# hebench/reference-seal-backend

Measured on AMD Instinct MI355X. Metric: ciphertext-ops/sec (CKKS ct x ct mul+relin+rescale, N=2^15, L=16), higher is better.
Workload: dtype u64 (exact residues; fp64-FMA engine for primes < 2^47, u64 Harvey engine with the fold reduction for the 60-bit primes)

## Files before the change

reference-seal-backend_amd/csrc/he355_kernels.hip:

```cpp
#include <hip/hip_runtime.h>

#include <cstdio>
#include <cstdlib>
#include <stdexcept>
#include <type_traits>

#include "he355_kernels.h"
#include "ntt_core.h"
#include "client/ckks_codec.h"
#include "client/multiword.h"
#include "client/sampler.h"

#if !defined(HE355_KNS) || !defined(HE355_U64_FOLD)
#error "he355_kernels.hip is compiled once per form of the u64 engine: -DHE355_KNS=ks_shoup -DHE355_U64_FOLD=0 and -DHE355_KNS=ks_fold -DHE355_U64_FOLD=1 (Makefile)"
#endif
namespace he355 {
namespace HE355_KNS {
namespace {

#include "kernel_common.inc"

template <class Ar>
__device__ __forceinline__ void rows_fwd_job(const PrimeDev &P, u64 *row, bool in_raw, u32 rowbase, int lane, u64 *lds, bool valid)
{
// ... 309 lines not shown
{
    s0 = s1 = s2 = make_ulonglong2(0, 0);
    for (int k = 0; k < inner; ++k, pa += a_step, pb += b_step) {
        const ulonglong2 a0 = reinterpret_cast<const ulonglong2 *>(pa)[e2], a1 = reinterpret_cast<const ulonglong2 *>(pa + P1)[e2];
        const ulonglong2 b0 = reinterpret_cast<const ulonglong2 *>(pb)[e2], b1 = reinterpret_cast<const ulonglong2 *>(pb + P1)[e2];
        ulonglong2 c0, c1, c2;
        mul3_pair(ar, a0, a1, b0, b1, c0, c1, c2);
        s0.x = addmod(s0.x, c0.x, q); s0.y = addmod(s0.y, c0.y, q);
        s1.x = addmod(s1.x, c1.x, q); s1.y = addmod(s1.y, c1.y, q);
        s2.x = addmod(s2.x, c2.x, q); s2.y = addmod(s2.y, c2.y, q);
    }
}

__global__ void __launch_bounds__(kBlock) k_mul3_acc(const u64 *a, const u64 *b, u64 *out, const PrimeDev *primes, int L, int logN, u64 rows, u64 cols,
                                                     int inner, u64 a_stride_i, u64 a_stride_k, u64 b_stride_k, u64 b_stride_j)
{
    const u64 pairs_per_poly = (u64)1 << (logN - 1);
    const u64 gid = (u64)blockIdx.x * kBlock + threadIdx.x;
    const u64 ri = gid >> (logN - 1);
    const u64 e2 = gid & (pairs_per_poly - 1);
    const u64 r = ri / L;
    if (r >= rows * cols) return;
    const int i = (int)(ri % L);
    const u64 poly = (u64)1 << logN, P1 = (u64)L << logN, ct = 2 * P1;
    const u64 *pa = a + (r / cols) * a_stride_i * ct + i * poly, *pb = b + (r % cols) * b_stride_j * ct + i * poly;
    ulonglong2 s0, s1, s2;
    const PrimeDev &P = primes[i];
    if (P.f64) mul3_acc_pair(make_ar(P, (ArF64 *)nullptr), P.q, pa, pb, a_stride_k * ct, b_stride_k * ct, P1, e2, inner, s0, s1, s2);
    else mul3_acc_pair(make_ar(P, (ArU64 *)nullptr), P.q, pa, pb, a_stride_k * ct, b_stride_k * ct, P1, e2, inner, s0, s1, s2);
    u64 *po = out + r * 3 * P1 + i * poly;
    reinterpret_cast<ulonglong2 *>(po)[e2] = s0;
    reinterpret_cast<ulonglong2 *>(po + P1)[e2] = s1;
    reinterpret_cast<ulonglong2 *>(po + 2 * P1)[e2] = s2;
}

template <class Ar, int BLOCK>
__device__ __forceinline__ typename std::conditional<std::is_same<Ar, ArF64>::value, TwRowF64, TwRow>::type
stage_row_twiddles(const PrimeDev &P, const Ar &ar, u32 rowbase, unsigned char *twl_raw, bool inverse = false)
{
    constexpr bool kF64 = std::is_same<Ar, ArF64>::value;
    typename std::conditional<kF64, TwRowF64, TwRow>::type twr;
    const gtw_t gf = gtw(inverse ? P.inv : P.fwd);
    constexpr int kIter = (kRowTw + BLOCK - 1) / BLOCK;
    Tw16 tmp[kIter];
#pragma unroll
    for (int k = 0; k < kIter; ++k) {
        const u32 i = threadIdx.x + k * BLOCK;
        tmp[k] = tw_load(gf, tw_row_source(rowbase, i + 1 < (u32)kRowTw ? i : 0));
    }
    if constexpr (kF64) {
        double *twl = reinterpret_cast<double *>(twl_raw);
#pragma unroll
        for (int k = 0; k < kIter; ++k)
            if (threadIdx.x + k * BLOCK < (u32)kRowTw) twl[threadIdx.x + k * BLOCK] = ArF64::tw_w(tmp[k]);
        twr.t = twl;
        twr.qinv = ar.qinv;
    } else {
        Tw16 *twl = reinterpret_cast<Tw16 *>(twl_raw);
#pragma unroll
        for (int k = 0; k < kIter; ++k)
            if (threadIdx.x + k * BLOCK < (u32)kRowTw) twl[threadIdx.x + k * BLOCK] = tmp[k];
        twr.t = twl;
    }
    return twr;
}

constexpr int K1_MUL_C2 = 3;
struct K1Args {
    const u64 *addend;
    const u64 *a, *b;
    Indexer ix;
    const uint32_t *perm;
    u64 *c01; u64 c01_item_stride;
    u64 *c2n, *c2r;
    u64 n_ops, op_offset;
    int L, logn1, mode;
    int no_c1;
    int no_c0n;
    int n_i;
    unsigned char i_list[64];
    KsGroups groups;
};

template <class Ar, int MODE, class ITW = int>
__device__ __forceinline__ void k1_job(const K1Args &A, const PrimeDev &P, u64 op, int i, u32 a_row, int lane, u64 *lds, bool valid, const ITW *staged = nullptr)
{
    typedef typename Ar::T T;
    const Ar ar = make_ar(P, (Ar *)nullptr);
    const u32 n1 = 1u << A.logn1;
    const u64 N = (u64)n1 << kRowLog, P1 = (u64)A.L * N;
    const u64 roff = (u64)i * N + ((u64)a_row << kRowLog);
    u64 *c0p = A.c01 + op * A.c01_item_stride + roff;
    u64 *c1p = c0p + P1;
    u64 *c2np = A.c2n + op * P1 + roff;
    u64 *c2rp = A.c2r + op * P1 + roff;
    T x[kRowE];
    u64 v0[kRowE], v1[kRowE];
    if (MODE == K1_MUL || MODE == K1_MUL_C2) {
        const u64 r = A.op_offset + op;
        const u64 *pa = A.a + idx_a(A.ix, r) * 2 * P1 + roff, *pb = A.b + idx_b(A.ix, r) * 2 * P1 + roff;
        u64 a0[kRowE], a1[kRowE], b0[kRowE], b1[kRowE];
        u64 v2[kRowE];
        if (MODE == K1_MUL_C2) {
            load_rowC(pa + P1, lane, a1);
            load_rowC(pb + P1, lane, b1);
#pragma unroll
            for (int r2 = 0; r2 < kRowE; ++r2) x[r2] = ar.dy_mul(ar.dy_in(a1[r2]), ar.dy_in(b1[r2]));
        } else {
        load_rowC(pa, lane, a0); load_rowC(pa + P1, lane, a1);
        load_rowC(pb, lane, b0); load_rowC(pb + P1, lane, b1);
#pragma unroll
        for (int r2 = 0; r2 < kRowE; ++r2) {
            const T x0 = ar.dy_in(a0[r2]), x1 = ar.dy_in(a1[r2]), y0 = ar.dy_in(b0[r2]), y1 = ar.dy_in(b1[r2]);
            v0[r2] = ar.dy_out(ar.dy_mul(x0, y0));
            v1[r2] = ar.dy_out(ar.dy_add(ar.dy_mul(x0, y1), ar.dy_mul(x1, y0)));
            v2[r2] = ar.dy_out(ar.dy_mul(x1, y1));
            x[r2] = ar.from_canon(v2[r2]);
        }
        if (valid) { store_rowC(c0p, lane, v0); store_rowC(c1p, lane, v1); store_rowC(c2np, lane, v2); }
        }
    } else if (MODE == K1_CT3) {
        const u64 *pa = A.a + (A.op_offset + op) * 3 * P1 + roff;
        u64 v2[kRowE];
        load_rowC(pa + 2 * P1, lane, v2);
#pragma unroll
        for (int r2 = 0; r2 < kRowE; ++r2) x[r2] = ar.from_canon(v2[r2]);
        if (!A.no_c1) {
            load_rowC(pa, lane, v0); load_rowC(pa + P1, lane, v1);
            if (valid) { store_rowC(c0p, lane, v0); store_rowC(c1p, lane, v1); store_rowC(c2np, lane, v2); }
        }
    } else {
        u64 src_ct = A.op_offset + op;
        const uint32_t *perm = A.perm;
        if (A.groups.group_size) {
            const u32 gop = (u32)(A.op_offset + op), grp = gop / A.groups.group_size;
            src_ct = (u64)A.groups.src_block[grp] * A.groups.group_size + gop % A.groups.group_size;
            perm = A.groups.perm[grp];
        }
        const u64 *p0 = A.a + src_ct * 2 * P1 + (u64)i * N;
        const uint32_t *pm = perm + ((u64)a_row << kRowLog);
        u64 v2[kRowE];
        {
            const u64 *srow = p0 + (u64)(__builtin_amdgcn_readfirstlane(pm[0]) & ~(u32)(kRowN - 1));
            u32 pl[kRowE];
#pragma unroll
            for (int r2 = 0; r2 < kRowE; ++r2) pl[r2] = lds_pad((int)(pm[elemC(lane, r2)] & (u32)(kRowN - 1)));
            u64 t[kRowE];
            load_rowC(srow + P1, lane, t);
            lds_store_C(lds, lane, t);
            HE_WAVE_SYNC();
#pragma unroll
            for (int r2 = 0; r2 < kRowE; ++r2) v2[r2] = lds[pl[r2]];
            if (!A.no_c0n) {
                load_rowC(srow, lane, t);
                HE_WAVE_SYNC();
                lds_store_C(lds, lane, t);
                HE_WAVE_SYNC();
#pragma unroll
                for (int r2 = 0; r2 < kRowE; ++r2) v0[r2] = lds[pl[r2]];
            }
            HE_WAVE_SYNC();
#pragma unroll
            for (int r2 = 0; r2 < kRowE; ++r2) {
                if (A.no_c0n) v0[r2] = 0;
                v1[r2] = 0;
                x[r2] = ar.from_canon(v2[r2]);
            }
        }
        if (A.addend && !A.no_c0n) {
            const u64 *ad = A.addend + (A.op_offset + op) * 2 * P1 + roff;
            u64 a0[kRowE];
            load_rowC(ad, lane, a0);
            if (!A.no_c1) load_rowC(ad + P1, lane, v1);
#pragma unroll
            for (int r2 = 0; r2 < kRowE; ++r2) v0[r2] = addmod(v0[r2], a0[r2], P.q);
        }
        if (valid) {
            if (!A.no_c0n) store_rowC(c0p, lane, v0);
            if (!A.no_c1) store_rowC(c1p, lane, v1);
            store_rowC(c2np, lane, v2);
        }
    }
    const bool last = A.logn1 == 0;
    if constexpr (std::is_same<ITW, int>::value) wave_rows_inv(ar, P, last, n1 + a_row, lane, lds, x);
    else wave_rows_inv_tw(ar, *staged, P.inv_w0_scaled, last, lane, lds, x);
#pragma unroll
    for (int r2 = 0; r2 < kRowE; ++r2) v0[r2] = last ? ar.to_canon(x[r2]) : ar.to_raw(x[r2]);
    if (valid) store_rowA(c2rp, lane, v0);
}

template <int MODE, class Ar>
__global__ void __launch_bounds__(kBlock) k_k1(K1Args A, const PrimeDev *primes)
{
    __shared__ u64 lds[kWaves][kLdsRow];
    constexpr bool kF64 = std::is_same<Ar, ArF64>::value;
    __shared__ __attribute__((aligned(16))) unsigned char twl_raw[kF64 ? kRowTw * 8 : kRowTw * 16];
    const int wave = threadIdx.x >> 6, lane = threadIdx.x & 63;
    const u32 n1 = 1u << A.logn1;
    const u64 n_opg = (A.n_ops + kWaves - 1) / kWaves;
    const u64 tile = blockIdx.x / n_opg, opg = blockIdx.x % n_opg;
    const u32 a_row = (u32)(tile & (n1 - 1));
    const int i = A.i_list[tile >> A.logn1];
    u64 op = opg * kWaves + wave;
    const bool valid = op < A.n_ops;
    if (!valid) op = A.n_ops - 1;
    const PrimeDev &P = primes[i];
    const Ar ar = make_ar(P, (Ar *)nullptr);
    const auto itw = stage_row_twiddles<Ar, kBlock>(P, ar, n1 + a_row, twl_raw, true);
    __syncthreads();
    k1_job<Ar, MODE>(A, P, op, i, a_row, lane, lds[wave], valid, &itw);
}
template <int MODE, class Ar>
__device__ __forceinline__ void k1_block(const K1Args &A, const PrimeDev *primes, const unsigned bid_x, u64 (*lds)[kLdsRow])
{
    const int wave = threadIdx.x >> 6, lane = threadIdx.x & 63;
    const u32 n1 = 1u << A.logn1;
    const u64 total = A.n_ops * A.n_i * n1;
    u64 job = (u64)bid_x * kWaves + wave;
    const bool valid = job < total;
    if (!valid) job = total - 1;
    const u32 a_row = (u32)(job & (n1 - 1));
    const u64 oi = job >> A.logn1;
    const int i = A.i_list[oi % A.n_i];
    const u64 op = oi / A.n_i;
    k1_job<Ar, MODE>(A, primes[i], op, i, a_row, lane, lds[wave], valid);
}
template <int MODE>
__global__ void __launch_bounds__(kBlock) k_k1_dual(K1Args AF, K1Args AU, unsigned n_f, const PrimeDev *primes)
{
    __shared__ u64 lds[kWaves][kLdsRow];
    if (blockIdx.x < n_f) k1_block<MODE, ArF64>(AF, primes, blockIdx.x, lds);
    else k1_block<MODE, ArU64>(AU, primes, blockIdx.x - n_f, lds);
}

struct K2Args {
    const u64 *c2r;
    u64 src_op_stride;
    u64 *d;
    u64 n_ops;
    int L, K, ckks, src_is_coeff;
    u64 f64_mask;
    int n_dig;
    unsigned char dig_list[64];
    int tsplit;
};

__device__ __forceinline__ double lift_wide(const ArF64 &ar, u64 v, double pow32)
{
    return ar.mulmod_vv((double)(u32)(v >> 32), pow32) + (double)(u32)v;
}
typedef const __attribute__((address_space(4))) double *cdw_t;
__device__ __forceinline__ cdw_t cdw(const double *p) { return (cdw_t)(unsigned long long)p; }
typedef u32 u32x2_t __attribute__((ext_vector_type(2)));
constexpr u32 kSlotBytes = kRowN * 8;
__device__ __forceinline__ __amdgpu_buffer_rsrc_t poly_rsrc(const void *p, u32 bytes)
{
    const unsigned long long v = (unsigned long long)p;
    const u32 lo = __builtin_amdgcn_readfirstlane((u32)v), hi = __builtin_amdgcn_readfirstlane((u32)(v >> 32));
    return __builtin_amdgcn_make_buffer_rsrc((void *)(((unsigned long long)hi << 32) | lo), 0, (int)bytes, 0x00020000);
}
template <int N1> __device__ __forceinline__ void store_pattern_rows(__amdgpu_buffer_rsrc_t dst, u32 off4, u32 off2h, const double x[N1])
{
#pragma unroll
    for (int a = 0; a < N1; ++a) {
        union { u64 u; double d; } c;
        c.d = x[a];
        __builtin_amdgcn_raw_buffer_store_b32((u32)c.u, dst, (int)off4, a * (int)kSlotBytes, 0);
        __builtin_amdgcn_raw_buffer_store_b16((unsigned short)(c.u >> 32), dst, (int)off2h, a * (int)kSlotBytes, 0);
    }
}
template <int N1> __device__ __forceinline__ void store_word_rows(__amdgpu_buffer_rsrc_t dst, u32 off8, const u64 x[N1])
{
#pragma unroll
    for (int a = 0; a < N1; ++a) {
        u32x2_t v;
        v.x = (u32)x[a]; v.y = (u32)(x[a] >> 32);
        __builtin_amdgcn_raw_buffer_store_b64(v, dst, (int)off8, a * (int)kSlotBytes, 0);
    }
}
typedef u32 u32x4_t __attribute__((ext_vector_type(4)));
template <int N1>
__device__ __forceinline__ void store_pattern_rows_wide(__amdgpu_buffer_rsrc_t dst, unsigned char *tile, int lane, u32 lane_lo, u32 lane_hi, const double x[N1])
{
    static_assert(N1 % 8 == 0, "written for whole groups of 8 rows");
    u32 *lo = reinterpret_cast<u32 *>(tile);
    unsigned short *hi = reinterpret_cast<unsigned short *>(tile + N1 * 256);
#pragma unroll
    for (int a = 0; a < N1; ++a) {
        union { u64 u; double d; } c;
        c.d = x[a];
        lo[a * 64 + lane] = (u32)c.u;
        hi[a * 64 + lane] = (unsigned short)(c.u >> 32);
    }
// ... 1802 lines not shown
```

reference-seal-backend_amd/csrc/k3_body.inc:

```
    static_assert(!GROUPED || !TENSOR, "grouped keys are for rotations");
    constexpr int kWaves = WAVES, kBlock = WAVES * 64;
    typedef typename Ar::T T;
    typedef typename Ar::Acc Acc;
    constexpr bool kF64 = std::is_same<Ar, ArF64>::value;
    constexpr bool kPacked = kF64;
    constexpr int kDigitPieces = kPacked ? 6 : 8;
    K3_LDS_DECL
    const int wave = threadIdx.x >> 6, lane = threadIdx.x & 63;
    const u32 n1 = 1u << A.logn1;
    const u64 N = (u64)n1 << kRowLog;
    const u64 n_og = (A.n_ops + kWaves - 1) / kWaves;
    const u64 n_ogb = (n_og + A.og_per_block - 1) / A.og_per_block;
    const u64 total_tiles = (u64)A.n_tt * n1;
    const u64 s = K3_BID_X >> 3, xcd = K3_BID_X & 7;
    const u64 tile = (s / n_ogb) * 8 + xcd;
    if (tile >= total_tiles) return;
    const u64 og_first = A.og_stride > 1 ? s % n_ogb : (s % n_ogb) * A.og_per_block;
    const int tt = A.tt_list[tile >> A.logn1];
    const int q_slot = A.q_slot[tile >> A.logn1];
    const u32 a_row = (u32)(tile & (n1 - 1));
    const int t = (tt == A.L) ? A.K - 1 : tt;
    const PrimeDev &P = primes[t];
    const Ar ar = make_ar(P, (Ar *)nullptr);
    const u64 rowoff = (u64)a_row << kRowLog;
    const auto twr = stage_row_twiddles<Ar, kBlock>(P, ar, n1 + a_row, twl_raw);
    __syncthreads();
    for (u32 g = 0; g < A.og_per_block; ++g) {
        const u64 og = og_first + (u64)g * A.og_stride;
        if (og >= n_og) break;
        u64 op = og * kWaves + wave;
        const bool valid = op < A.n_ops;
        if (!valid) op = A.n_ops - 1;
        Acc acc0[kRowE], acc1[kRowE];
#pragma unroll
        for (int r = 0; r < kRowE; ++r) { acc0[r] = 0; acc1[r] = 0; }
        auto tensor_init = [&]() {
            if constexpr (TENSOR) {
                const u64 tr = A.t_op_offset + op;
                const u64 LNt = (u64)A.L * N;
                const u64 *pa = A.ta + idx_a(A.tix, tr) * 2 * LNt + (u64)tt * N + rowoff;
                const u64 *pb = A.tb + idx_b(A.tix, tr) * 2 * LNt + (u64)tt * N + rowoff;
                u64 a0[kRowE], a1[kRowE], b0[kRowE], b1[kRowE];
                load_rowC(pa, lane, a0); load_rowC(pb, lane, b0);
                load_rowC(pa + LNt, lane, a1); load_rowC(pb + LNt, lane, b1);
#pragma unroll
                for (int r = 0; r < kRowE; ++r) {
                    const T x0 = ar.dy_in(a0[r]), x1 = ar.dy_in(a1[r]), y0 = ar.dy_in(b0[r]), y1 = ar.dy_in(b1[r]);
                    acc0[r] = ar.acc_from_lazy(ar.dy_mul(x0, y0));
                    acc1[r] = ar.acc_from_lazy(ar.dy_add(ar.dy_mul(x0, y1), ar.dy_mul(x1, y0)));
                }
            }
        };
        constexpr int kRun = Ar::kAccRun;
        int pend = 0;
        auto acc_flush = [&]() {
            if constexpr (kRun > 1) {
                if (pend) {
#pragma unroll
                    for (int r = 0; r < kRowE; ++r) { acc0[r] = ar.acc_reduce(acc0[r]); acc1[r] = ar.acc_reduce(acc1[r]); }
                    pend = 0;
                }
            }
        };
        auto acc_step = [&]() {
            if constexpr (kRun > 1) {
                if (++pend == kRun) acc_flush();
            }
        };
        auto mac_row = [&](Acc acc[kRowE], const T x[kRowE], const u64 kv[kRowE], const u64 kq[kRowE]) {
#pragma unroll
            for (int r = 0; r < kRowE; ++r) {
                if constexpr (kRun > 1) ar.acc_mac_lazy(acc[r], x[r], ar.key_in(kv[r]), Ar::kKeyQuotient ? kq[r] : 0);
                else ar.acc_mac(acc[r], x[r], ar.key_in(kv[r]), Ar::kKeyQuotient ? kq[r] : 0);
            }
        };
        const u64 *kbase = A.key, *kqbase = A.keyq;
        if constexpr (GROUPED) {
            typedef const __attribute__((address_space(4))) unsigned long long *ckeys_t;
            const u32 grp = __builtin_amdgcn_readfirstlane((u32)((A.g_op_offset + op) / A.groups.group_size));
            kbase = (const u64 *)((ckeys_t)(unsigned long long)A.groups.key)[grp];
            kqbase = kbase + A.keyq_offset;
        }
        auto key_row = [&](int j, int k) -> const u64 * { return kbase + (((u64)j * 2 + k) * A.K + t) * N + rowoff; };
        auto keyq_row = [&](int j, int k) -> const u64 * { return kqbase + (((u64)j * 2 + k) * A.n_q + q_slot) * N + rowoff; };
        auto mac_poly = [&](Acc acc[kRowE], const T x[kRowE], int j, int k) {
            u64 kv[kRowE], kq[kRowE];
            load_rowC(key_row(j, k), lane, kv);
            if constexpr (Ar::kKeyQuotient) load_rowC(keyq_row(j, k), lane, kq);
            mac_row(acc, x, kv, kq);
        };
        auto mac_digit = [&](const T x[kRowE], int j) {
            mac_poly(acc0, x, j, 0);
            mac_poly(acc1, x, j, 1);
            acc_step();
        };
        auto gather_base = [&](int poly, const uint32_t *&pm) -> const u64 * {
            u64 src_ct = A.gsrc_op_offset + op;
            pm = A.gperm;
            if constexpr (GROUPED) {
                const u32 gop = (u32)(A.g_op_offset + op), gi = __builtin_amdgcn_readfirstlane(gop / A.groups.group_size);
                src_ct = (u64)A.groups.src_block[gi] * A.groups.group_size + gop % A.groups.group_size;
                pm = A.groups.perm[gi];
            }
            pm += rowoff;
            return A.gsrc + (src_ct * 2 + (u64)poly) * ((u64)A.L * N) + (u64)tt * N;
        };
        auto gather_row = [&](int poly, u64 v[kRowE]) {
            const uint32_t *pm;
            const u64 *p0 = gather_base(poly, pm);
#pragma unroll
            for (int r = 0; r < kRowE; ++r) v[r] = p0[pm[elemC(lane, r)]];
        };
        const bool has_own = A.ckks && tt < A.L;
        const int nd = A.L - (has_own ? 1 : 0);
        auto digit = [&](int i) -> int { return (has_own && i >= tt) ? i + 1 : i; };
        const int split = FUSE ? 1 : (A.n_split > 1 ? A.n_split : 1), grp = split > 1 ? (int)K3_BID_Y : 0;
        const int i_begin = nd * grp / split, i_end = nd * (grp + 1) / split;
        auto src_row = [&](int j) -> const u64 * { return A.d + ((op * (A.L + 1) + tt) * A.L + j) * N + rowoff; };
        if (i_begin < i_end) dma_row_to_lds<kDigitPieces>(src_row(digit(i_begin)), stage[wave], lane);
        tensor_init();
        if (has_own && grp == 0) {
            if constexpr (TENSOR) {
                const u64 tr = A.t_op_offset + op;
                const u64 LNt = (u64)A.L * N;
                u64 a1[kRowE], b1[kRowE];
                load_rowC(A.ta + (idx_a(A.tix, tr) * 2 + 1) * LNt + (u64)tt * N + rowoff, lane, a1);
                load_rowC(A.tb + (idx_b(A.tix, tr) * 2 + 1) * LNt + (u64)tt * N + rowoff, lane, b1);
                T x[kRowE];
#pragma unroll
                for (int r = 0; r < kRowE; ++r) x[r] = ar.dy_mul(ar.dy_in(a1[r]), ar.dy_in(b1[r]));
                mac_digit(x, tt);
            } else {
                T x[kRowE];
                u64 v[kRowE];
                load_rowC(FUSE && A.c1_mode == 3 ? A.c1_src + (op * 3 + 2) * ((u64)A.L * N) + (u64)tt * N + rowoff : A.c2n + (op * A.L + tt) * N + rowoff, lane, v);
#pragma unroll
                for (int r = 0; r < kRowE; ++r) x[r] = ar.from_canon(v[r]);
                mac_digit(x, tt);
            }
        }
        if constexpr (FUSE || TENSOR) {
            const bool resc = A.cols2 != nullptr;
            const int n_rows = nd + 2;
            const u64 LN = (u64)A.L * N, L1N = (u64)(A.L - 1) * N;
            auto row_ptr = [&](int i) -> const u64 * {
                if (i < nd) return src_row(digit(i));
                if (!resc) return A.cols + ((op * 2 + (i - nd)) * A.L + tt) * N + rowoff;
                return A.cols2 + ((op * 2 + (i - nd)) * (A.L - 1) + tt) * N + rowoff;
            };
            const FloorConst fc = A.fc[(A.K - 1) * A.K + t];
            const FloorConst fc2 = A.fc[(resc ? A.L - 1 : 0) * A.K + t];
            if (FUSE && nd == 0) dma_row_to_lds(row_ptr(0), stage[wave], lane);
            for (int i = 0; i < nd; ++i) {
                T x[1][kRowE];
                asm volatile("s_waitcnt vmcnt(0)" ::: "memory");
                if constexpr (kPacked) {
                    lds_rowA48(stage[wave], lane, x[0]);
                } else {
                    u64 v[kRowE];
                    lds_rowA(stage[wave], lane, v);
#pragma unroll
                    for (int r = 0; r < kRowE; ++r) x[0][r] = ar.from_raw(v[r]);
                }
                asm volatile("s_waitcnt lgkmcnt(0)" ::: "memory");
                if (i + 1 < nd) dma_row_to_lds<kDigitPieces>(row_ptr(i + 1), stage[wave], lane);
                else if constexpr (FUSE) dma_row_to_lds(row_ptr(i + 1), stage[wave], lane);
                if constexpr (!Ar::kKeyQuotient) {
                    u64 kv0[kRowE], kv1[kRowE];
                    const int j = digit(i);
                    wave_rows_fwd_n(ar, twr, lane, lds[wave], x, [&]() { load_rowC(key_row(j, 0), lane, kv0); load_rowC(key_row(j, 1), lane, kv1); });
                    if constexpr (kF64) {
#pragma unroll
                        for (int r0 = 0; r0 < kRowE; r0 += kMacG / 2) {
                            double xs[kMacG], ks[kMacG], pr[kMacG];
#pragma unroll
                            for (int k = 0; k < kMacG / 2; ++k) {
                                xs[2 * k] = x[0][r0 + k]; ks[2 * k] = ar.key_in(kv0[r0 + k]);
                                xs[2 * k + 1] = x[0][r0 + k]; ks[2 * k + 1] = ar.key_in(kv1[r0 + k]);
                            }
                            ar.template mulmod_vv_g<kMacG>(xs, ks, pr);
#pragma unroll
                            for (int k = 0; k < kMacG / 2; ++k) { acc0[r0 + k] += pr[2 * k]; acc1[r0 + k] += pr[2 * k + 1]; }
                        }
                    }
                } else {
                    wave_rows_fwd_n<Ar, decltype(twr), NoHook, true>(ar, twr, lane, lds[wave], x);
                    mac_digit(x[0], digit(i));
                }
            }
            acc_flush();
            constexpr bool kAccForms = TENSOR || GROUPED;
            const bool direct = kAccForms && Ar::kAccDirect && floor_direct(P.acc_terms, (u32)A.L + 2);
#pragma unroll 1
            for (int i = nd; FUSE && i < n_rows; ++i) {
                T x[1][kRowE];
                u64 v[kRowE], av[kRowE];
                asm volatile("s_waitcnt vmcnt(0)" ::: "memory");
                lds_rowA(stage[wave], lane, v);
#pragma unroll
                for (int r = 0; r < kRowE; ++r) x[0][r] = ar.from_raw(v[r]);
                asm volatile("s_waitcnt lgkmcnt(0)" ::: "memory");
                if (i + 1 < n_rows) dma_row_to_lds(row_ptr(i + 1), stage[wave], lane);
                const int k = i - nd;
                u64 *c01_row = A.c01 + op * A.c01_item_stride + k * LN + (u64)tt * N + rowoff;
                if constexpr (TENSOR) {
                } else if (k == 0 && A.c1_mode == 4) {
                    gather_row(0, av);
                } else if (k == 0 && A.c1_mode == 5) {
                    u64 ad[kRowE];
                    load_rowC(A.c1_src + (op * 2 + 0) * LN + (u64)tt * N + rowoff, lane, ad);
                    gather_row(0, av);
#pragma unroll
                    for (int r = 0; r < kRowE; ++r) av[r] = addmod(av[r], ad[r], P.q);
                } else if (k == 1 && (A.c1_mode == 1 || A.c1_mode == 4)) {
#pragma unroll
                    for (int r = 0; r < kRowE; ++r) av[r] = 0;
                } else if (A.c1_mode == 3) {
                    load_rowC(A.c1_src + (op * 3 + k) * LN + (u64)tt * N + rowoff, lane, av);
                } else {
                    load_rowC(k == 1 && (A.c1_mode == 2 || A.c1_mode == 5) ? A.c1_src + (op * 2 + 1) * LN + (u64)tt * N + rowoff : c01_row, lane, av);
                }
                bool into_sum = false;
                u64 *sum_row = nullptr;
                u32 sum_cnt = 0;
                if constexpr (GROUPED && !TENSOR) {
                    if (A.groups.sum_out) {
                        const u32 gop = (u32)(A.g_op_offset + op), gi = __builtin_amdgcn_readfirstlane(gop / A.groups.group_size);
                        sum_cnt = A.groups.count[gi];
                        sum_row = A.groups.sum_out + ((u64)(gop % A.groups.group_size) * 2 + k) * LN + (u64)tt * N + rowoff;
                        into_sum = sum_cnt == 1 && !resc;
                        if (into_sum) {
                            u64 o[kRowE];
                            load_rowC(sum_row, lane, o);
#pragma unroll
                            for (int r = 0; r < kRowE; ++r) av[r] = addmod(av[r], o[r], P.q);
                        }
                    }
                }
                if constexpr (!kF64 && Ar::kFold) {
                    wave_rows_fwd_n<Ar, decltype(twr), NoHook, true>(ar, twr, lane, lds[wave], x);
#pragma unroll
                    for (int r = 0; r < kRowE; ++r) x[0][r] = ar.lazy_reduce(x[0][r]);
                } else {
                    wave_rows_fwd_n(ar, twr, lane, lds[wave], x);
                }
                const Acc *acc = k == 0 ? acc0 : acc1;
                if (kAccForms && Ar::kAccDirect && !direct) {
                    if (k == 0) {
#pragma unroll
                        for (int r = 0; r < kRowE; ++r) ar.floor_prep(acc0[r], x[0][r]);
                    } else {
#pragma unroll
                        for (int r = 0; r < kRowE; ++r) ar.floor_prep(acc1[r], x[0][r]);
                    }
                }
                if constexpr (TENSOR) {
                    if (!resc) {
#pragma unroll
                        for (int r = 0; r < kRowE; ++r) v[r] = ar.floor_fin_s_acc(acc[r], x[0][r], fc.inv, fc.inv_shoup, fc.inv_d, fc.inv_i);
                        if (valid) store_rowC(c01_row, lane, v);
                    } else {
#pragma unroll
                        for (int r = 0; r < kRowE; ++r) v[r] = ar.floor_fin2_s_acc(acc[r], x[0][r], fc2);
                        if (valid) store_rowC(A.out2 + (op * 2 + k) * L1N + (u64)tt * N + rowoff, lane, v);
                    }
                } else if (!resc) {
#pragma unroll
                    for (int r = 0; r < kRowE; ++r) {
                        if constexpr (kAccForms) v[r] = ar.floor_fin_acc(acc[r], x[0][r], fc.inv, fc.inv_shoup, fc.inv_d, fc.inv_i, av[r]);
                        else v[r] = ar.floor_fin(ar.acc_canon(acc[r]), x[0][r], fc.inv, fc.inv_shoup, fc.inv_d, fc.inv_i, av[r]);
                    }
                    if constexpr (GROUPED) {
                        if (into_sum) {
                            if (valid) store_rowC(sum_row, lane, v);
                        } else if (A.groups.sum_out) {
// ... 82 lines not shown
```

reference-seal-backend_amd/csrc/modarith.h:

```cpp
#pragma once
#include <cstdint>

#if defined(__HIP__)
#define HE_HD __host__ __device__ inline __attribute__((always_inline))
#else
#define HE_HD inline
#endif

#if defined(__HIP_DEVICE_COMPILE__)
#define HE_SCHED_FENCE() __builtin_amdgcn_sched_barrier(0)
#else
#define HE_SCHED_FENCE() ((void)0)
#endif

namespace he355 {

#if defined(HE355_LANE_SIM)
extern int he355_sim_overflow;
#endif

typedef uint64_t u64;
typedef uint32_t u32;
typedef unsigned __int128 u128;

// ... 34 lines not shown
{
    u64 r = mul_shoup_lazy(x, w, wq, q);
    return r >= q ? r - q : r;
}

constexpr u64 kFoldMask60 = 0x0FFFFFFFFFFFFFFFull, kFoldMask61 = 0x1FFFFFFFFFFFFFFFull;
constexpr u32 kFoldMaxC = 1u << 26;
HE_HD bool fold_prime_ok(u64 q) { return (q >> 59) == 1 && (q >> 60) == 0 && ((u64)1 << 60) - q < kFoldMaxC; }
HE_HD u32 fold_c(u64 q) { return (u32)(((u64)1 << 60) - q); }
HE_HD u64 fold_sum(u64 x, u64 w, u64 w2, u32 &lo)
{
    const u32 x0 = (u32)x, x1 = (u32)(x >> 32);
    const u64 u = (u64)x0 * (u32)w;
    const u64 u2 = (u64)x1 * (u32)w2 + (u32)u;
    const u64 m1 = (u64)x0 * (u32)(w >> 32) + (u >> 32);
    const u64 m2 = (u64)x1 * (u32)(w2 >> 32) + (u2 >> 32);
    lo = (u32)u2;
    return m1 + m2;
}
HE_HD u64 fold_mul_tight(u64 x, u64 w, u64 w2, u32 c)
{
    u32 lo;
    const u64 up = fold_sum(x, w, w2, lo);
    const u32 h = (u32)(up >> 29), b = (u32)(up >> 28) & 1u;
    const u64 lo60 = ((up & 0x0FFFFFFFull) << 32) | lo;
    return (u64)h * (2 * c) + ((u64)b * c + lo60);
}
HE_HD u64 fold_mul_wide(u64 x, u64 w, u64 w2, u32 c)
{
    u32 lo;
    const u64 up = fold_sum(x, w, w2, lo);
    const u32 h = (u32)(up >> 29);
    const u64 lo61 = ((up & 0x1FFFFFFFull) << 32) | lo;
    return (u64)h * (2 * c) + lo61;
}
HE_HD u64 fold_red2q(u64 x, u32 c) { return (x & kFoldMask61) + (u64)(u32)(x >> 61) * (2 * c); }
HE_HD u64 fold_acc128(u128 acc, u64 q, u32 c)
{
    const u64 lo = (u64)acc & kFoldMask60;
    const u128 hc = (acc >> 60) * c;
    const u64 l2 = (u64)hc & kFoldMask60, h2 = (u64)(hc >> 60);
    u64 r = h2 * c + lo + l2;
    r = (r & kFoldMask60) + (r >> 60) * c;
    return r >= q ? r - q : r;
}

struct alignas(16) Tw16 {
    u64 a, b;
};

#ifndef HE355_U64_FOLD
#define HE355_U64_FOLD 0
#endif
#if HE355_U64_FOLD
#define HE355_ARITH_NS u64_fold_form
#else
#define HE355_ARITH_NS u64_shoup_form
#endif
inline namespace HE355_ARITH_NS {
#if HE355_U64_FOLD
HE_HD u64 mul_pre_lazy(u64 x, u64 w, u64 w2, u64 q) { return fold_mul_tight(x, w, w2, fold_c(q)); }
#else
HE_HD u64 mul_pre_lazy(u64 x, u64 w, u64 w2, u64 q) { return mul_shoup_lazy(x, w, w2, q); }
#endif
HE_HD u64 mul_pre(u64 x, u64 w, u64 w2, u64 q)
{
    const u64 r = mul_pre_lazy(x, w, w2, q);
    return r >= q ? r - q : r;
}
HE_HD u64 pre_word(u64 w, u64 q, bool fold) { return fold ? (u64)(((u128)w << 32) % q) : (u64)(((u128)w << 64) / q); }

struct ArU64 {
    typedef u64 T;
    u64 q, two_q;
    u64 ninv, ninv_q;
    u64 cr0, cr1;
    static constexpr bool kFold = HE355_U64_FOLD != 0;
    HE_HD u32 c() const { return fold_c(q); }

    HE_HD ModU64 mod() const { ModU64 m; m.q = q; m.cr0 = cr0; m.cr1 = cr1; return m; }
    HE_HD T dy_in(u64 c) const { return c; }
    HE_HD T dy_mul(T x, T y) const { return barrett128((u128)x * y, mod()); }
    HE_HD T dy_add(T x, T y) const { return addmod(x, y, q); }
    HE_HD u64 dy_out(T x) const { return x; }
    HE_HD T key_in(u64 bits) const { return bits; }
    typedef u64 Acc;
#if HE355_U64_FOLD
    static constexpr bool kKeyQuotient = true;
    static constexpr int kAccRun = 5;
    HE_HD void acc_mac_lazy(Acc &acc, T x, T key, u64 key2) const
    {
        const u64 v = fold_mul_wide(x, key, key2, c());
#if defined(HE355_LANE_SIM)
        if (acc > ~(u64)0 - v) he355_sim_overflow = 1;
#endif
        acc += v;
    }
    HE_HD void acc_mac(Acc &acc, T x, T key, u64 key2) const { acc = fold_red2q(acc + fold_mul_wide(x, key, key2, c()), c()); }
    HE_HD Acc acc_reduce(Acc acc) const { return fold_red2q(acc, c()); }
    HE_HD u64 acc_canon(Acc acc) const { return to_canon(fold_red2q(acc, c())); }
    HE_HD Acc acc_from_canon(u64 v) const { return v; }
    HE_HD Acc acc_from_lazy(T v) const { return v; }
#else
    static constexpr bool kKeyQuotient = true;
    HE_HD void acc_mac(Acc &acc, T x, T key, u64 keyq) const
    {
        const u64 s = acc + mul_pre_lazy(x, key, keyq, q);
        acc = s >= 2 * two_q ? s - 2 * two_q : s;
    }
    static constexpr int kAccRun = 6;
    HE_HD void acc_mac_lazy(Acc &acc, T x, T key, u64 keyq) const
    {
        const u64 v = mul_pre_lazy(x, key, keyq, q);
#if defined(HE355_LANE_SIM)
        if (acc > ~(u64)0 - v) he355_sim_overflow = 1;
#endif
        acc += v;
    }
    HE_HD Acc acc_reduce(Acc acc) const { return reduce16_to_4q(acc); }
    HE_HD u64 acc_canon(Acc acc) const { return to_canon(acc); }
    HE_HD Acc acc_from_canon(u64 v) const { return v; }
    HE_HD Acc acc_from_lazy(T v) const { return v; }
#endif
    HE_HD u64 shoup_quotient_est(u64 w) const { return w * cr1 + mulhi64(w, cr0); }
    HE_HD u64 shoup_quotient(u64 w) const
    {
        u64 est = shoup_quotient_est(w);
        u64 r = 0 - est * q;
        if (r >= q) { r -= q; ++est; }
        if (r >= q) { r -= q; ++est; }
        return est;
    }
    HE_HD u64 floor_fin(u64 t, T x, u64 inv, u64 inv_shoup, double, double, u64 addend) const
    {
        u64 r = mul_pre(t + 2 * two_q - x, inv, inv_shoup, q);
        return addmod(r, addend, q);
    }

    template <class FC> HE_HD u64 floor_fin2(u64 t, T x, const FC &f1, const FC &f2, u64 addend) const
    {
        const u64 r1 = mul_pre(t, f1.inv, f1.inv_shoup, q);
        return mul_pre(r1 + addend + 2 * two_q - x, f2.inv, f2.inv_shoup, q);
    }
    HE_HD u64 floor_fin_s(u64 t, T x, u64 inv, u64 inv_shoup, double, double) const { return submod(t, mul_pre(x, inv, inv_shoup, q), q); }
    template <class FC> HE_HD u64 floor_fin2_s(u64 t, T x, const FC &f2) const { return mul_pre(t + 2 * two_q - x, f2.inv, f2.inv_shoup, q); }
    static constexpr bool kAccDirect = false;
    HE_HD void floor_prep(Acc &, T &) const {}
    HE_HD u64 floor_fin_acc(Acc acc, T x, u64 inv, u64 inv_shoup, double inv_d, double inv_i, u64 addend) const
    {
        return floor_fin(acc_canon(acc), x, inv, inv_shoup, inv_d, inv_i, addend);
    }
    template <class FC> HE_HD u64 floor_fin2_acc(Acc acc, T x, const FC &f1, const FC &f2, u64 addend) const { return floor_fin2(acc_canon(acc), x, f1, f2, addend); }
    HE_HD u64 floor_fin_s_acc(Acc acc, T x, u64 inv, u64 inv_shoup, double inv_d, double inv_i) const
    {
        return floor_fin_s(acc_canon(acc), x, inv, inv_shoup, inv_d, inv_i);
    }
    template <class FC> HE_HD u64 floor_fin2_s_acc(Acc acc, T x, const FC &f2) const { return floor_fin2_s(acc_canon(acc), x, f2); }
    HE_HD T acc_to_inv(Acc acc) const { return from_canon(acc_canon(acc)); }
    HE_HD u64 acc_park(Acc acc) const { return acc_canon(acc); }
    HE_HD T acc_unpark(u64 w) const { return from_canon(w); }
    HE_HD T from_canon(u64 x) const { return x; }
    HE_HD T from_raw(u64 bits) const { return bits; }
    HE_HD u64 to_raw(T x) const { return x; }
    HE_HD u64 to_canon(T x) const
    {
        if (x >= two_q) x -= two_q;
// ... 102 lines not shown
HE_HD u64 f64_to_u52(double x)
{
    union { u64 u; double d; } c;
    c.d = x + 4503599627370496.0;
    return c.u & 0x000FFFFFFFFFFFFFull;
}

struct ArF64 {
    typedef double T;
    double q, qinv;
    double ninv, ninv_i;

    HE_HD T from_canon(u64 x) const { return u52_to_f64(x); }
    HE_HD T from_raw(u64 bits) const
    {
        union { u64 u; double d; } c;
        c.u = bits;
        return c.d;
    }
    HE_HD u64 to_raw(T x) const
    {
        union { u64 u; double d; } c;
        c.d = x;
        return c.u;
    }
    HE_HD T canon(T x) const
    {
        double c = __builtin_floor(x * qinv);
        double r = __builtin_fma(-c, q, x);
        if (r < 0.0) r += q;
        if (r >= q) r -= q;
        return r;
    }
    HE_HD u64 to_canon(T x) const { return f64_to_u52(canon(x)); }
    HE_HD T mulmod_c(T y, double w, double winv) const
    {
        double h = y * w;
        double l = __builtin_fma(y, w, -h);
        double c = __builtin_rint(y * winv);
        double d = __builtin_fma(-c, q, h);
        return d + l;
    }
    HE_HD T mulmod_vv(T x, T y) const
    {
        double h = x * y;
        double l = __builtin_fma(x, y, -h);
        double c = __builtin_rint(h * qinv);
        double d = __builtin_fma(-c, q, h);
        return d + l;
    }
    template <int G> HE_HD void mulmod_vv_g(const T (&x)[G], const T (&y)[G], T (&out)[G]) const
    {
        double h[G], l[G], c[G];
#pragma unroll
        for (int k = 0; k < G; ++k) h[k] = x[k] * y[k];
        HE_SCHED_FENCE();
#pragma unroll
        for (int k = 0; k < G; ++k) c[k] = h[k] * qinv;
#pragma unroll
        for (int k = 0; k < G; ++k) l[k] = __builtin_fma(x[k], y[k], -h[k]);
        HE_SCHED_FENCE();
#pragma unroll
        for (int k = 0; k < G; ++k) c[k] = __builtin_rint(c[k]);
        HE_SCHED_FENCE();
#pragma unroll
        for (int k = 0; k < G; ++k) h[k] = __builtin_fma(-c[k], q, h[k]);
        HE_SCHED_FENCE();
#pragma unroll
        for (int k = 0; k < G; ++k) out[k] = h[k] + l[k];
        HE_SCHED_FENCE();
    }
    HE_HD T canon2(T x) const
    {
        if (x < 0.0) x += q;
        if (x < 0.0) x += q;
        if (x >= q) x -= q;
        return x;
    }
    HE_HD u64 to_canon2(T x) const { return f64_to_u52(canon2(x)); }
    typedef double Acc;
    HE_HD T dy_in(u64 c) const { return u52_to_f64(c); }
    HE_HD T dy_mul(T x, T y) const { return mulmod_vv(x, y); }
    HE_HD T dy_add(T x, T y) const { return x + y; }
    HE_HD u64 dy_out(T x) const { return to_canon2(x); }
    HE_HD T key_in(u64 bits) const { return from_raw(bits); }
    static constexpr bool kKeyQuotient = false;
    HE_HD void acc_mac(Acc &acc, T x, T key, u64) const { acc += mulmod_vv(x, key); }
    static constexpr int kAccRun = 1;
    HE_HD void acc_mac_lazy(Acc &acc, T x, T key, u64) const { acc += mulmod_vv(x, key); }
    HE_HD Acc acc_reduce(Acc acc) const { return acc; }
    HE_HD u64 acc_canon(Acc acc) const { return to_canon(acc); }
    HE_HD Acc acc_from_canon(u64 v) const { return u52_to_f64(v); }
    HE_HD Acc acc_from_lazy(T v) const { return v; }
    HE_HD u64 floor_fin(u64 t, T x, u64, u64, double inv_d, double inv_i, u64 addend) const
    {
        double m = mulmod_c(u52_to_f64(t) - x, inv_d, inv_i);
        return to_canon2(m + u52_to_f64(addend));
    }
    template <class FC> HE_HD u64 floor_fin2(u64 t, T x, const FC &f1, const FC &f2, u64 addend) const
    {
        const double m1 = mulmod_c(u52_to_f64(t), f1.inv_d, f1.inv_i);
        return to_canon2(mulmod_c(m1 + u52_to_f64(addend) - x, f2.inv_d, f2.inv_i));
    }
    HE_HD u64 floor_fin_s(u64 t, T x, u64, u64, double inv_d, double inv_i) const { return to_canon2(u52_to_f64(t) - mulmod_c(x, inv_d, inv_i)); }
    template <class FC> HE_HD u64 floor_fin2_s(u64 t, T x, const FC &f2) const { return to_canon2(mulmod_c(u52_to_f64(t) - x, f2.inv_d, f2.inv_i)); }
    static constexpr bool kAccDirect = true;
    HE_HD void floor_prep(Acc &acc, T &x) const
    {
        acc = renorm(acc);
        x = renorm(x);
    }
    HE_HD T canon_neg(T x) const { return x < 0.0 ? x + q : x; }
    HE_HD T canon_1(T x) const
    {
        if (x < 0.0) x += q;
        if (x >= q) x -= q;
        return x;
    }
    HE_HD u64 floor_fin_acc(Acc acc, T x, u64, u64, double inv_d, double inv_i, u64 addend) const
    {
        return f64_to_u52(canon_1(mulmod_c(acc - x, inv_d, inv_i) + u52_to_f64(addend)));
    }
    template <class FC> HE_HD u64 floor_fin2_acc(Acc acc, T x, const FC &f1, const FC &f2, u64 addend) const
    {
        const double m1 = mulmod_c(acc, f1.inv_d, f1.inv_i);
        return f64_to_u52(canon_neg(mulmod_c(m1 + u52_to_f64(addend) - x, f2.inv_d, f2.inv_i)));
    }
    HE_HD u64 floor_fin_s_acc(Acc acc, T x, u64, u64, double inv_d, double inv_i) const
    {
        return f64_to_u52(canon_neg(renorm(acc - mulmod_c(x, inv_d, inv_i))));
    }
    template <class FC> HE_HD u64 floor_fin2_s_acc(Acc acc, T x, const FC &f2) const { return f64_to_u52(canon_neg(mulmod_c(acc - x, f2.inv_d, f2.inv_i))); }
    HE_HD T acc_to_inv(Acc acc) const { return renorm(acc); }
    HE_HD u64 acc_park(Acc acc) const { return to_raw(renorm(acc)); }
    HE_HD T acc_unpark(u64 w) const { return from_raw(w); }
    HE_HD static double tw_w(const Tw16 &t)
    {
        union { u64 u; double d; } c;
        c.u = t.a;
        return c.d;
    }
    HE_HD static double tw_wi(const Tw16 &t)
    {
        union { u64 u; double d; } c;
        c.u = t.b;
        return c.d;
    }
    template <bool SW = false> HE_HD void bfly_fwd(T &X, T &Y, const Tw16 &w) const
    {
        double t = mulmod_vv(Y, tw_w(w));
        double x = X;
        X = x + t;
        Y = x - t;
    }
    template <int G> HE_HD void bfly_fwd_g(T (&X)[G], T (&Y)[G], const Tw16 (&w)[G]) const
    {
        double h[G], l[G], c[G];
#pragma unroll
        for (int k = 0; k < G; ++k) h[k] = Y[k] * tw_w(w[k]);
        HE_SCHED_FENCE();
#pragma unroll
        for (int k = 0; k < G; ++k) c[k] = h[k] * qinv;
#pragma unroll
        for (int k = 0; k < G; ++k) l[k] = __builtin_fma(Y[k], tw_w(w[k]), -h[k]);
        HE_SCHED_FENCE();
#pragma unroll
        for (int k = 0; k < G; ++k) c[k] = __builtin_rint(c[k]);
        HE_SCHED_FENCE();
#pragma unroll
        for (int k = 0; k < G; ++k) h[k] = __builtin_fma(-c[k], q, h[k]);
        HE_SCHED_FENCE();
#pragma unroll
        for (int k = 0; k < G; ++k) l[k] = h[k] + l[k];
        HE_SCHED_FENCE();
#pragma unroll
        for (int k = 0; k < G; ++k) {
            Y[k] = X[k] - l[k];
            X[k] = X[k] + l[k];
        }
        HE_SCHED_FENCE();
    }
    template <int G, bool SW = false> HE_HD void bfly_fwd_lazy_g(T (&X)[G], T (&Y)[G], const Tw16 (&w)[G]) const { bfly_fwd_g<G>(X, Y, w); }
    HE_HD T reduce16_to_4q(T x) const { return x; }
    static constexpr bool kFold = false;
    HE_HD T lazy_reduce(T x) const { return x; }
    template <bool SW = false> HE_HD void bfly_inv(T &X, T &Y, const Tw16 &w) const
    {
        double s = X + Y;
        double d = X - Y;
        X = s;
        Y = mulmod_vv(d, tw_w(w));
    }
    template <bool SW = false> HE_HD void bfly_inv_last(T &X, T &Y, const Tw16 &w_scaled) const
    {
        double s = X + Y;
        double d = X - Y;
        X = mulmod_c(s, ninv, ninv_i);
        Y = mulmod_c(d, tw_w(w_scaled), tw_wi(w_scaled));
    }
    HE_HD T scale_ninv(T x) const { return mulmod_c(x, ninv, ninv_i); }
    HE_HD T renorm(T x) const { return __builtin_fma(-__builtin_rint(x * qinv), q, x); }
    static constexpr bool kNeedsRenormInv = true;
};

constexpr double kFloorAccMax = 562949953421312.0, kFloorXMax = 562949953421312.0;
HE_HD double f64_stage_growth(double m, double q, int stages)
{
    for (int s = 0; s < stages; ++s) m += q * (0.5 + m * 4.440892098500626e-16);
    return m;
}
HE_HD double floor_term_bound(u64 q)
{
    const double qd = (double)q;
    return qd * (0.5 + f64_stage_growth(140737488355328.0, qd, 10) * 4.440892098500626e-16);
}
HE_HD u32 floor_direct_terms(u64 q)
{
    const double qd = (double)q;
    if (q >> 47) return 0;
    if (!(f64_stage_growth(4.0 * qd, qd, 15) <= kFloorXMax)) return 0;
    const double t = kFloorAccMax / floor_term_bound(q);
    return t >= 4294967295.0 ? 0xFFFFFFFFu : (u32)t;
}
HE_HD bool floor_direct(u32 acc_terms, u32 terms) { return terms <= acc_terms; }

}
```

Before: 23280.

## Use Karatsuba tensor product and reuse c2 in key-switch; prefetch c2 rows in k1

In the fused tensor+keyswitch kernel, the degree-2 ciphertext product now uses a Karatsuba-style three-multiply form (c0, c2, and (a0+a1)(b0+b1)-c0-c2). The c2 term is kept in registers and fed straight into the own-digit MAC, so the a1/b1 rows are no longer reloaded and multiplied a second time. The direct-floor bound check is widened to account for the extra accumulated terms of the lazy f64 result. The K1_MUL_C2 kernel also issues its a1/b1 row loads before twiddle staging and the barrier, so the loads overlap with that work. Risks: the f64 Karatsuba result is less reduced, which may push some primes off the direct floor path, and register pressure rises.

```diff
diff --git a/reference-seal-backend_amd/csrc/he355_kernels.hip b/reference-seal-backend_amd/csrc/he355_kernels.hip
--- a/reference-seal-backend_amd/csrc/he355_kernels.hip
+++ b/reference-seal-backend_amd/csrc/he355_kernels.hip
@@ -415,8 +415,21 @@
     KsGroups groups;
 };
 
+struct K1RowsC2 {
+    u64 a1[kRowE], b1[kRowE];
+};
+__device__ __forceinline__ void k1_load_rows_c2(const K1Args &A, u64 op, int i, u32 a_row, int lane, K1RowsC2 &R)
+{
+    const u64 N = (u64)(1u << A.logn1) << kRowLog, P1 = (u64)A.L * N;
+    const u64 roff = (u64)i * N + ((u64)a_row << kRowLog);
+    const u64 r = A.op_offset + op;
+    load_rowC(A.a + (idx_a(A.ix, r) * 2 + 1) * P1 + roff, lane, R.a1);
+    load_rowC(A.b + (idx_b(A.ix, r) * 2 + 1) * P1 + roff, lane, R.b1);
+}
+
 template <class Ar, int MODE, class ITW = int>
-__device__ __forceinline__ void k1_job(const K1Args &A, const PrimeDev &P, u64 op, int i, u32 a_row, int lane, u64 *lds, bool valid, const ITW *staged = nullptr)
+__device__ __forceinline__ void k1_job(const K1Args &A, const PrimeDev &P, u64 op, int i, u32 a_row, int lane, u64 *lds, bool valid, const ITW *staged = nullptr,
+                                       const K1RowsC2 *rows_c2 = nullptr)
 {
     typedef typename Ar::T T;
     const Ar ar = make_ar(P, (Ar *)nullptr);
@@ -435,10 +448,8 @@
         u64 a0[kRowE], a1[kRowE], b0[kRowE], b1[kRowE];
         u64 v2[kRowE];
         if (MODE == K1_MUL_C2) {
-            load_rowC(pa + P1, lane, a1);
-            load_rowC(pb + P1, lane, b1);
-#pragma unroll
-            for (int r2 = 0; r2 < kRowE; ++r2) x[r2] = ar.dy_mul(ar.dy_in(a1[r2]), ar.dy_in(b1[r2]));
+#pragma unroll
+            for (int r2 = 0; r2 < kRowE; ++r2) x[r2] = ar.dy_mul(ar.dy_in(rows_c2->a1[r2]), ar.dy_in(rows_c2->b1[r2]));
         } else {
         load_rowC(pa, lane, a0); load_rowC(pa + P1, lane, a1);
         load_rowC(pb, lane, b0); load_rowC(pb + P1, lane, b1);
@@ -539,9 +550,17 @@
     if (!valid) op = A.n_ops - 1;
     const PrimeDev &P = primes[i];
     const Ar ar = make_ar(P, (Ar *)nullptr);
-    const auto itw = stage_row_twiddles<Ar, kBlock>(P, ar, n1 + a_row, twl_raw, true);
-    __syncthreads();
-    k1_job<Ar, MODE>(A, P, op, i, a_row, lane, lds[wave], valid, &itw);
+    if constexpr (MODE == K1_MUL_C2) {
+        K1RowsC2 rows;
+        k1_load_rows_c2(A, op, i, a_row, lane, rows);
+        const auto itw = stage_row_twiddles<Ar, kBlock>(P, ar, n1 + a_row, twl_raw, true);
+        __syncthreads();
+        k1_job<Ar, MODE>(A, P, op, i, a_row, lane, lds[wave], valid, &itw, &rows);
+    } else {
+        const auto itw = stage_row_twiddles<Ar, kBlock>(P, ar, n1 + a_row, twl_raw, true);
+        __syncthreads();
+        k1_job<Ar, MODE>(A, P, op, i, a_row, lane, lds[wave], valid, &itw);
+    }
 }
 template <int MODE, class Ar>
 __device__ __forceinline__ void k1_block(const K1Args &A, const PrimeDev *primes, const unsigned bid_x, u64 (*lds)[kLdsRow])
diff --git a/reference-seal-backend_amd/csrc/k3_body.inc b/reference-seal-backend_amd/csrc/k3_body.inc
--- a/reference-seal-backend_amd/csrc/k3_body.inc
+++ b/reference-seal-backend_amd/csrc/k3_body.inc
@@ -34,7 +34,7 @@
         Acc acc0[kRowE], acc1[kRowE];
 #pragma unroll
         for (int r = 0; r < kRowE; ++r) { acc0[r] = 0; acc1[r] = 0; }
-        auto tensor_init = [&]() {
+        auto tensor_init = [&](T c2[kRowE]) {
             if constexpr (TENSOR) {
                 const u64 tr = A.t_op_offset + op;
                 const u64 LNt = (u64)A.L * N;
@@ -45,9 +45,10 @@
                 load_rowC(pa + LNt, lane, a1); load_rowC(pb + LNt, lane, b1);
 #pragma unroll
                 for (int r = 0; r < kRowE; ++r) {
-                    const T x0 = ar.dy_in(a0[r]), x1 = ar.dy_in(a1[r]), y0 = ar.dy_in(b0[r]), y1 = ar.dy_in(b1[r]);
-                    acc0[r] = ar.acc_from_lazy(ar.dy_mul(x0, y0));
-                    acc1[r] = ar.acc_from_lazy(ar.dy_add(ar.dy_mul(x0, y1), ar.dy_mul(x1, y0)));
+                    T p0, p1;
+                    ar.dy_mul3(ar.dy_in(a0[r]), ar.dy_in(a1[r]), ar.dy_in(b0[r]), ar.dy_in(b1[r]), p0, p1, c2[r]);
+                    acc0[r] = ar.acc_from_lazy(p0);
+                    acc1[r] = ar.acc_from_lazy(p1);
                 }
             }
         };
@@ -118,18 +119,11 @@
         const int i_begin = nd * grp / split, i_end = nd * (grp + 1) / split;
         auto src_row = [&](int j) -> const u64 * { return A.d + ((op * (A.L + 1) + tt) * A.L + j) * N + rowoff; };
         if (i_begin < i_end) dma_row_to_lds<kDigitPieces>(src_row(digit(i_begin)), stage[wave], lane);
-        tensor_init();
+        T c2[kRowE];
+        tensor_init(c2);
         if (has_own && grp == 0) {
             if constexpr (TENSOR) {
-                const u64 tr = A.t_op_offset + op;
-                const u64 LNt = (u64)A.L * N;
-                u64 a1[kRowE], b1[kRowE];
-                load_rowC(A.ta + (idx_a(A.tix, tr) * 2 + 1) * LNt + (u64)tt * N + rowoff, lane, a1);
-                load_rowC(A.tb + (idx_b(A.tix, tr) * 2 + 1) * LNt + (u64)tt * N + rowoff, lane, b1);
-                T x[kRowE];
-#pragma unroll
-                for (int r = 0; r < kRowE; ++r) x[r] = ar.dy_mul(ar.dy_in(a1[r]), ar.dy_in(b1[r]));
-                mac_digit(x, tt);
+                mac_digit(c2, tt);
             } else {
                 T x[kRowE];
                 u64 v[kRowE];
@@ -190,7 +184,7 @@
             }
             acc_flush();
             constexpr bool kAccForms = TENSOR || GROUPED;
-            const bool direct = kAccForms && Ar::kAccDirect && floor_direct(P.acc_terms, (u32)A.L + 2);
+            const bool direct = kAccForms && Ar::kAccDirect && floor_direct(P.acc_terms, (u32)A.L + (TENSOR ? kTensorTerms : 2u));
 #pragma unroll 1
             for (int i = nd; FUSE && i < n_rows; ++i) {
                 T x[1][kRowE];
diff --git a/reference-seal-backend_amd/csrc/modarith.h b/reference-seal-backend_amd/csrc/modarith.h
--- a/reference-seal-backend_amd/csrc/modarith.h
+++ b/reference-seal-backend_amd/csrc/modarith.h
@@ -140,6 +140,12 @@
     HE_HD T dy_in(u64 c) const { return c; }
     HE_HD T dy_mul(T x, T y) const { return barrett128((u128)x * y, mod()); }
     HE_HD T dy_add(T x, T y) const { return addmod(x, y, q); }
+    HE_HD void dy_mul3(T a0, T a1, T b0, T b1, T &c0, T &c1, T &c2) const
+    {
+        c0 = dy_mul(a0, b0);
+        c2 = dy_mul(a1, b1);
+        c1 = submod(submod(dy_mul(addmod(a0, a1, q), addmod(b0, b1, q)), c0, q), c2, q);
+    }
     HE_HD u64 dy_out(T x) const { return x; }
     HE_HD T key_in(u64 bits) const { return bits; }
     typedef u64 Acc;
@@ -408,6 +414,12 @@
     HE_HD T dy_in(u64 c) const { return u52_to_f64(c); }
     HE_HD T dy_mul(T x, T y) const { return mulmod_vv(x, y); }
     HE_HD T dy_add(T x, T y) const { return x + y; }
+    HE_HD void dy_mul3(T a0, T a1, T b0, T b1, T &c0, T &c1, T &c2) const
+    {
+        c0 = mulmod_vv(a0, b0);
+        c2 = mulmod_vv(a1, b1);
+        c1 = mulmod_vv(a0 + a1, b0 + b1) - c0 - c2;
+    }
     HE_HD u64 dy_out(T x) const { return to_canon2(x); }
     HE_HD T key_in(u64 bits) const { return from_raw(bits); }
     static constexpr bool kKeyQuotient = false;
@@ -530,6 +542,7 @@
 };
 
 constexpr double kFloorAccMax = 562949953421312.0, kFloorXMax = 562949953421312.0;
+constexpr unsigned kTensorTerms = 3;
 HE_HD double f64_stage_growth(double m, double q, int stages)
 {
     for (int s = 0; s < stages; ++s) m += q * (0.5 + m * 4.440892098500626e-16);
```

After: 23600 (median of 6 runs). 1.4% higher.
